# nz0001na/MorphGANformer

Measured on AMD Instinct MI355X. Metric: latent-projection iters/sec @1024^2, k=17 latents, higher is better.
Workload: dtype f32; 1 GPU; configs[1]: single 1024x1024 face per GPU, Wing+LPIPS(squeeze)+MSE literal-mode projection step, noise_mode=random, seeded synthetic weights/targets/landmarks; k=17, z_dim=32, targets_per_gpu=1, parallelism=pair-sharded x1, graph_replay=True, loss_generator_overlap=True, steps_per_forward=32

## Files before the change

include/mgf.h:

```cpp
#ifndef MGF_H_
#define MGF_H_

#include <stdint.h>

#ifdef __cplusplus
extern "C" {
#endif

typedef void* mgf_stream_t;

enum { MGF_OK = 0, MGF_EINVAL = -1, MGF_EUNSUPPORTED = -2, MGF_ELAUNCH = -3, MGF_ETOOBIG = -4 };
enum { MGF_F32 = 0, MGF_F64 = 1, MGF_F16 = 2 };
enum { MGF_FILTER_SEPARABLE = 2 };
enum { MGF_FILTER_LARGE = 4 };
enum { MGF_ACT_LINEAR = 1, MGF_ACT_RELU = 2, MGF_ACT_LRELU = 3, MGF_ACT_TANH = 4, MGF_ACT_SIGMOID = 5,
       MGF_ACT_ELU = 6, MGF_ACT_SELU = 7, MGF_ACT_SOFTPLUS = 8, MGF_ACT_SWISH = 9,
       MGF_ACT_RELU_POST = 10 };

const char* mgf_last_error(void);
int mgf_version(void);
int mgf_device_ok(void);

int mgf_bias_act(void* y, const void* x, const void* b, const void* xref, const void* yref, const void* dy,
                 int dtype, int64_t numel, int64_t step_b, int64_t size_b,
// ... 66 lines not shown
                                  const float* rgb_w, const float* rgb_bias, int32_t n, int32_t cin, int32_t h, int32_t w, int32_t cout,
                                  int32_t out_scale_stride, int32_t rgb_channels, mgf_stream_t stream);
int mgf_conv3x3_winograd2_f32(float* y, const float* x, const float* u, const float* in_scale, const float* out_scale, int32_t n,
                              int32_t cin, int32_t h, int32_t w, int32_t cout, int32_t out_scale_stride, const mgf_epilogue* ep,
                              mgf_stream_t stream);
int mgf_conv3x3_winograd3_f32(float* y, const float* x, const float* u, const float* in_scale, const float* out_scale, int32_t n,
                              int32_t cin, int32_t h, int32_t w, int32_t cout, int32_t out_scale_stride, const mgf_epilogue* ep,
                              mgf_stream_t stream);
int mgf_conv3x3_winograd3_slice_f32(float* y, const float* x, const float* u, const float* in_scale, const float* out_scale, int32_t n,
                                    int32_t cin, int32_t h, int32_t w, int32_t cout, int32_t out_scale_stride, int64_t y_batch,
                                    int32_t y_choff, const mgf_epilogue* ep, mgf_stream_t stream);
int mgf_conv1x1_f32(float* y, const float* x, const float* w, const float* in_scale, int32_t n, int32_t cin, int32_t hw, int32_t cout,
                    int32_t cout_pad, int64_t y_batch, int32_t y_choff, const mgf_epilogue* ep, mgf_stream_t stream);
int mgf_conv1x1_force_shape(int32_t channel_blocks);

int mgf_conv3x3s2_few_inputs_f32(float* y, const float* x, const float* w, const float* bias, int32_t n, int32_t cin, int32_t in_h,
                                 int32_t in_w, int32_t cout, int32_t relu, mgf_stream_t stream);
int mgf_tconv3x3s2_few_outputs_f32(float* y, const float* x, const float* wp, int32_t n, int32_t cin, int32_t h, int32_t w, int32_t cout,
                                   int32_t cout_pad, int32_t pitch, int64_t y_plane, int64_t y_batch, mgf_stream_t stream);
int mgf_conv3x3_winograd3_up2res_f32(float* y, const float* x, const float* u, const float* in_scale, const float* out_scale,
                                     const float* residual_low, int32_t n, int32_t cin, int32_t h, int32_t w, int32_t cout,
                                     int32_t out_scale_stride, const mgf_epilogue* ep, mgf_stream_t stream);
int mgf_winograd3_force_shape(int32_t shape);
int mgf_conv3x3_winograd3_rgb_f32(float* rgb_out, const float* x, const float* u, const float* in_scale, const float* out_scale,
                                  const float* rgb_w, const float* rgb_bias, int32_t n, int32_t cin, int32_t h, int32_t w, int32_t cout,
                                  int32_t out_scale_stride, int32_t rgb_channels, mgf_stream_t stream);
int mgf_conv3x3_winograd_f32(float* y, const float* x, const float* u, const float* in_scale, const float* out_scale, int32_t n,
                             int32_t cin, int32_t h, int32_t w, int32_t cout, int32_t out_scale_stride, const mgf_epilogue* ep,
                             mgf_stream_t stream);

int mgf_tconv3x3s2_border_f32(float* t, const float* x, const float* wp, const float* in_scale, const float* out_scale, int32_t n,
                              int32_t cin, int32_t h, int32_t w, int32_t cout, int32_t cout_pad, int64_t t_pitch, int64_t t_plane,
                              int64_t t_batch, int64_t out_scale_stride, mgf_stream_t stream);

int mgf_tconv3x3s2_winograd_f32(float* t, const float* x, const float* u, const float* in_scale, const float* out_scale, int32_t n,
                                int32_t cin, int32_t h, int32_t w, int32_t cout, int32_t pitch, int64_t t_plane, int64_t t_batch,
                                int64_t out_scale_stride, mgf_stream_t stream);
int mgf_tconv_winograd_weights_f32(float* u, const float* w, int32_t cout, int32_t cin, double gain, mgf_stream_t stream);

int mgf_pack_conv_weights(float* wp, float* wsq, const float* w, int32_t cout, int32_t cin, int32_t kh, int32_t kw,
                          int32_t cout_pad, float gain, int32_t flip, mgf_stream_t stream);

typedef struct mgf_style_job {
    const float* aff_w;
    const float* aff_b;
    const float* wsq;
    float* s;
    float* d;
    int32_t cin, cout;
    int32_t w_offset;
    float aff_gain, style_gain;
} mgf_style_job;
int mgf_demod_f32(float* d, const float* s, const float* wsq, int32_t n, int32_t cin, int32_t cout, mgf_stream_t stream);
int mgf_demod_bwd_f32(float* ds, const float* dd, const float* d, const float* s, const float* wsq, int32_t n, int32_t cin, int32_t cout,
                      mgf_stream_t stream);
int mgf_style_demod(const mgf_style_job* job, const float* ws, int64_t ws_stride_n, int32_t n, int32_t wdim, mgf_stream_t stream);
int mgf_style_demod_multi(const mgf_style_job* jobs_dev, int32_t njobs, const float* ws, int64_t ws_stride_n,
                          int32_t n, int32_t wdim, int32_t max_cin, mgf_stream_t stream);

int mgf_duplex_attention(float* y, const float* x, const float* wqc, const float* spos, const float* vwb,
                         int32_t n, int32_t c, int32_t f, int32_t t,
                         const mgf_epilogue* ep, int32_t ep_w, float* probs, int32_t* argmax, mgf_stream_t stream);

int mgf_att_map_upsample_f32(float* out, const float* probs, int32_t n, int32_t side, int32_t t, int32_t out_res, int32_t layer,
                             int32_t n_layers, mgf_stream_t stream);

// ... 226 lines not shown
```

morphganformer_amd/_lib.py:

```python
from __future__ import annotations

import ctypes as C
import os

import torch

HERE = os.path.dirname(os.path.abspath(__file__))
LIB_PATH = os.environ.get("MGF_LIB_PATH") or os.path.join(HERE, "libmgf_hip.so")

MGF_F32, MGF_F64, MGF_F16 = 0, 1, 2
ACT_IDS = {"linear": 1, "relu": 2, "lrelu": 3, "tanh": 4, "sigmoid": 5, "elu": 6, "selu": 7, "softplus": 8, "swish": 9,
           "relu_post": 10}
MAX_TAPS = 9

i32, i64, f32, f64, vp = C.c_int32, C.c_int64, C.c_float, C.c_double, C.c_void_p


class Epilogue(C.Structure):
    _fields_ = [("bias", vp), ("noise", vp), ("noise_strength", vp), ("noise_n", i32), ("act", i32), ("alpha", f32),
                ("gain", f32), ("residual", vp)]


class ConvDesc(C.Structure):
    _fields_ = [("n", i32), ("cin", i32), ("in_h", i32), ("in_w", i32), ("cout", i32), ("cout_pad", i32),
# ... 11 lines not shown
class StyleJob(C.Structure):
    _fields_ = [("aff_w", vp), ("aff_b", vp), ("wsq", vp), ("s", vp), ("d", vp), ("cin", i32), ("cout", i32),
                ("w_offset", i32), ("aff_gain", f32), ("style_gain", f32)]


class AttnJob(C.Structure):
    _fields_ = [("wmv", vp), ("bmv", vp), ("vwb", vp), ("c", i32), ("w_offset", i32)]


class StyleBwdJob(C.Structure):
    _fields_ = [("aff_w", vp), ("wsq", vp), ("s", vp), ("d", vp), ("ds_part", vp), ("dc_part", vp), ("cin", i32), ("cout", i32),
                ("s_chunks", i32), ("d_chunks", i32), ("aff_gain", f32), ("style_gain", f32)]


class AttnGradJob(C.Structure):
    _fields_ = [("dg", vp), ("probs", vp), ("dc", vp), ("cpre", vp), ("part", vp), ("dvwb", vp), ("dc_part", vp), ("c", i32), ("f", i32),
                ("slices", i32), ("nchunk", i32), ("blk_grad", i32), ("blk_dot", i32), ("blk_red", i32), ("pad_", i32)]


class AttnBwdJob(C.Structure):
    _fields_ = [("wmv", vp), ("dvwb", vp), ("c", i32), ("pad_", i32)]


_SIGS = {
    "mgf_last_error": (C.c_char_p, []),
    "mgf_version": (C.c_int, []),
    "mgf_device_ok": (C.c_int, []),
    "mgf_bias_act": (C.c_int, [vp, vp, vp, vp, vp, vp, C.c_int, i64, i64, i64, C.c_int, C.c_int, f32, f32, f32, vp]),
    "mgf_upfirdn2d": (C.c_int, [vp, vp, vp, C.c_int, i32, i32, i32, i32, i64, i64, i64, i64, i32, i32, i64, i64, i64, i64,
                                i32, i32, i32, i32, i32, i32, i32, i32, i32, i32, i32, f32, C.POINTER(Epilogue), vp]),
    "mgf_conv_taps_f32": (C.c_int, [vp, vp, vp, vp, vp, C.POINTER(ConvDesc), C.POINTER(Epilogue), vp]),
    "mgf_conv_taps_bf16x3_f32": (C.c_int, [vp, vp, vp, vp, vp, C.POINTER(ConvDesc), C.POINTER(Epilogue), vp]),
    "mgf_tconv3x3s2_border_f32": (C.c_int, [vp, vp, vp, vp, vp, i32, i32, i32, i32, i32, i32, i64, i64, i64, i64, vp]),
    "mgf_tconv3x3s2_winograd_f32": (C.c_int, [vp, vp, vp, vp, vp, i32, i32, i32, i32, i32, i32, i64, i64, i64, vp]),
    "mgf_tconv_winograd_weights_f32": (C.c_int, [vp, vp, i32, i32, C.c_double, vp]),
    "mgf_winograd_weights_f32": (C.c_int, [vp, vp, i32, i32, f32, vp]),
    "mgf_conv3x3_winograd_f32": (C.c_int, [vp, vp, vp, vp, vp, i32, i32, i32, i32, i32, i32, C.POINTER(Epilogue), vp]),
    "mgf_winograd2_weights_f32": (C.c_int, [vp, vp, i32, i32, f32, vp]),
    "mgf_conv3x3_winograd2_f32": (C.c_int, [vp, vp, vp, vp, vp, i32, i32, i32, i32, i32, i32, C.POINTER(Epilogue), vp]),
    "mgf_conv3x3_winograd2_rgb_f32": (C.c_int, [vp, vp, vp, vp, vp, vp, vp, i32, i32, i32, i32, i32, i32, i32, vp]),
    "mgf_conv3x3_winograd3_f32": (C.c_int, [vp, vp, vp, vp, vp, i32, i32, i32, i32, i32, i32, C.POINTER(Epilogue), vp]),
    "mgf_conv1x1_f32": (C.c_int, [vp, vp, vp, vp, i32, i32, i32, i32, i32, i64, i32, C.POINTER(Epilogue), vp]),
    "mgf_conv3x3s2_few_inputs_f32": (C.c_int, [vp, vp, vp, vp, i32, i32, i32, i32, i32, i32, vp]),
    "mgf_tconv3x3s2_few_outputs_f32": (C.c_int, [vp, vp, vp, i32, i32, i32, i32, i32, i32, i32, i64, i64, vp]),
    "mgf_conv1x1_force_shape": (C.c_int, [i32]),
    "mgf_conv3x3_winograd3_slice_f32": (C.c_int, [vp, vp, vp, vp, vp, i32, i32, i32, i32, i32, i32, i64, i32, C.POINTER(Epilogue), vp]),
    "mgf_conv3x3_winograd3_up2res_f32": (C.c_int, [vp, vp, vp, vp, vp, vp, i32, i32, i32, i32, i32, i32, C.POINTER(Epilogue), vp]),
    "mgf_winograd3_force_shape": (C.c_int, [i32]),
    "mgf_conv3x3_winograd3_rgb_f32": (C.c_int, [vp, vp, vp, vp, vp, vp, vp, i32, i32, i32, i32, i32, i32, i32, vp]),
    "mgf_conv3x3_winograd2_slice_f32": (C.c_int, [vp, vp, vp, vp, vp, i32, i32, i32, i32, i32, i32, i64, i32, C.POINTER(Epilogue), vp]),
    "mgf_pack_conv_weights": (C.c_int, [vp, vp, vp, i32, i32, i32, i32, i32, f32, i32, vp]),
    "mgf_conv_profile_begin": (C.c_int, []),
    "mgf_conv_profile_end": (C.c_int, [C.POINTER(ConvProfRec), i32]),
    "mgf_demod_f32": (C.c_int, [vp, vp, vp, i32, i32, i32, vp]),
    "mgf_demod_bwd_f32": (C.c_int, [vp, vp, vp, vp, vp, i32, i32, i32, vp]),
    "mgf_style_demod": (C.c_int, [C.POINTER(StyleJob), vp, i64, i32, i32, vp]),
    "mgf_style_demod_multi": (C.c_int, [vp, i32, vp, i64, i32, i32, i32, vp]),
    "mgf_duplex_attention": (C.c_int, [vp, vp, vp, vp, vp, i32, i32, i32, i32, C.POINTER(Epilogue), i32, vp, vp, vp]),
    "mgf_att_map_upsample_f32": (C.c_int, [vp, vp, i32, i32, i32, i32, i32, i32, vp]),
    "mgf_attn_values": (C.c_int, [C.POINTER(AttnJob), vp, i64, i64, i32, i32, i32, vp]),
    "mgf_attn_values_multi": (C.c_int, [vp, i32, vp, i64, i64, i32, i32, i32, vp]),
    "mgf_randn_f32": (C.c_int, [vp, i64, C.c_uint64, vp, vp]),
    "mgf_rgb_weights_f32": (C.c_int, [vp, vp, vp, i32, i32, i32, vp]),
    "mgf_torgb_compose_weights_f32": (C.c_int, [vp, vp, vp, vp, vp, vp, i32, i32, i32, i32, vp]),
    "mgf_conv3x3_few_outputs_f32": (C.c_int, [vp, vp, vp, vp, i32, i32, i32, i32, i32, vp]),
    "mgf_mapping_param_floats": (i64, [i32, i32, i32]),
# ... 151 lines not shown
```

morphganformer_amd/build.py:

```python
from __future__ import annotations

import glob
import hashlib
import os
import subprocess
import sys

HERE = os.path.dirname(os.path.abspath(__file__))
ROOT = os.path.dirname(HERE)
CSRC = os.path.join(HERE, "csrc")
OBJ = os.path.join(CSRC, "_obj")
LIB = os.path.join(HERE, "libmgf_hip.so")
SOURCES = ["capi.cpp", "bias_act.hip", "upfirdn2d.hip", "conv_taps.hip", "latent_prep.hip", "attention.hip", "losses.hip", "lpips_stem.hip",
           "embed.hip", "backward.hip", "wino.hip", "wino3.hip", "pointwise.hip", "narrow_conv.hip", "warp.hip", "lbp.hip", "mdf.hip",
           "wino_tconv.hip", "depthwise.hip", "noise_opt.hip", "morph_pair.hip"]
HEADERS = [os.path.join(CSRC, "mgf_common.h"), os.path.join(ROOT, "include", "mgf.h")]
HIPCC = os.environ.get("HIPCC", "/opt/rocm/bin/hipcc")
FLAGS = ["--offload-arch=gfx950", "-O3", "-fPIC", "-std=c++17", "-ffp-contract=on", "-Wno-unused-result", "-x", "hip"]
LINK_FLAGS = ["--offload-arch=gfx950", "-shared", "-fPIC"]

_compiler_id = None


def compiler_id() -> str:
    global _compiler_id
    if _compiler_id is None:
        _compiler_id = subprocess.run([HIPCC, "--version"], stdout=subprocess.PIPE, stderr=subprocess.STDOUT, check=True).stdout.decode()
    return _compiler_id


def object_key(src_path: str, flags) -> str:
    h = hashlib.sha256()
    h.update(compiler_id().encode())
    h.update("\0".join(flags).encode())
    for p in [src_path] + HEADERS:
        with open(p, "rb") as f:
            h.update(b"\0" + os.path.basename(p).encode() + b"\0" + f.read())
    return h.hexdigest()[:16]


def _compile_all(obj_dir, flags_for, verbose, force, prune=True):
    os.makedirs(obj_dir, exist_ok=True)
    objs, todo = [], []
    for src in SOURCES:
        sp = os.path.join(CSRC, src)
        flags = flags_for(src)
        op = os.path.join(obj_dir, f"{src}.{object_key(sp, flags)}.o")
        objs.append(op)
# ... 95 lines not shown
```

morphganformer_amd/conv.py:

```python
from __future__ import annotations

import ctypes as C
import os
from dataclasses import dataclass

import torch

from . import _lib


def round_up(v: int, m: int) -> int:
    return (v + m - 1) // m * m


def profile_begin():
    _lib.check(_lib.lib().mgf_conv_profile_begin(), "conv_profile_begin")


def profile_end(max_recs=4096):
    recs = (_lib.ConvProfRec * max_recs)()
    n = _lib.lib().mgf_conv_profile_end(recs, max_recs)
    if n < 0:
        _lib.check(n, "conv_profile_end")
    return [(recs[i].kernel.decode(), recs[i].flops, recs[i].seconds, recs[i].ksplit, recs[i].bytes) for i in range(min(n, max_recs))]
# ... 407 lines not shown
        _lib.check(rc, "tconv3x3s2_few_outputs")
        return out[:, :, :, :ow]
    if wt is not None and tconv_winograd_ok(n, cin, h, w, pc.cout, out, bf):
        assert tuple(wt.shape) == (25, cin // 4, pc.cout, 4)
        os_stride = 0 if out_scale is None else out_scale.stride(0) if out_scale.ndim == 2 else 0
        rc = _lib.lib().mgf_tconv3x3s2_winograd_f32(out.data_ptr(), x.data_ptr(), wt.data_ptr(), _lib.ptr(in_scale), _lib.ptr(out_scale), n, cin, h,
                                                    w, pc.cout, pitch, oh * pitch, pc.cout * oh * pitch, os_stride, _lib.stream_ptr())
        _lib.check(rc, "tconv3x3s2_winograd")
        rc = _lib.lib().mgf_tconv3x3s2_border_f32(out.data_ptr(), x.data_ptr(), pc.wp.data_ptr(), _lib.ptr(in_scale), _lib.ptr(out_scale),
                                                  n, cin, h, w, pc.cout, pc.cout_pad, pitch, oh * pitch, pc.cout * oh * pitch, os_stride,
                                                  _lib.stream_ptr())
        _lib.check(rc, "tconv3x3s2_border")
        return out[:, :, :, :ow]
    split = SPLIT_TCONV_BORDER and min(h, w) >= (TCONV_SPLIT_MIN if n >= 4 else max(TCONV_SPLIT_MIN, 128))
    use_bf = bf is not None and split and w % 32 == 0 and cin % 16 == 0
    os_stride = 0 if out_scale is None else out_scale.stride(0) if out_scale.ndim == 2 else 0
    d = _desc(n, cin, h, w, pc.cout, pc.cout_pad, h if split else h + 1, w if split else w + 1, 1, 2, TCONV_TAPS, TCONV_GROUPS,
              [0, 0, 1, 1], [0, 1, 0, 1], oh, ow, pitch, oh * pitch, pc.cout * oh * pitch, 0, os_stride)
    if use_bf:
        rc = _lib.lib().mgf_conv_taps_bf16x3_f32(out.data_ptr(), x.data_ptr(), bf.data_ptr(), _lib.ptr(in_scale), _lib.ptr(out_scale),
                                                 C.byref(d), None, _lib.stream_ptr())
    else:
        rc = _lib.lib().mgf_conv_taps_f32(out.data_ptr(), x.data_ptr(), pc.wp.data_ptr(), _lib.ptr(in_scale), _lib.ptr(out_scale),
                                          C.byref(d), None, _lib.stream_ptr())
    _lib.check(rc, "conv_taps(tconv)")
    if split:
        rc = _lib.lib().mgf_tconv3x3s2_border_f32(out.data_ptr(), x.data_ptr(), pc.wp.data_ptr(), _lib.ptr(in_scale), _lib.ptr(out_scale),
                                                  n, cin, h, w, pc.cout, pc.cout_pad, pitch, oh * pitch, pc.cout * oh * pitch, os_stride,
                                                  _lib.stream_ptr())
        _lib.check(rc, "tconv3x3s2_border")
    return out[:, :, :, :ow]


def upfirdn_into(y, x, f2d, up=1, pad=(0, 0, 0, 0), gain=1.0, flip=False, epilogue=None, separable=False, down=1):
    _lib.require_gpu(x, y, f2d)
    n, c, h, w = x.shape
    fh, fw = f2d.shape
    px0, px1, py0, py1 = pad
    oh = (h * up + py0 + py1 - fh + down) // down
    ow = (w * up + px0 + px1 - fw + down) // down
    assert tuple(y.shape) == (n, c, oh, ow), (tuple(y.shape), (n, c, oh, ow))
    sx, sy = x.stride(), y.stride()
    rc = _lib.lib().mgf_upfirdn2d(y.data_ptr(), x.data_ptr(), f2d.data_ptr(), _lib.MGF_F32, n, c, h, w, sx[0], sx[1], sx[2],
                                  sx[3], oh, ow, sy[0], sy[1], sy[2], sy[3], fh, fw, up, up, down, down, px0, px1, py0, py1,
                                  int(flip) | (2 if separable else 0) | 4,
                                  float(gain), C.byref(epilogue) if epilogue is not None else None,
                                  _lib.stream_ptr())
    _lib.check(rc, "upfirdn2d")
    return y
```

morphganformer_amd/engine.py:

```python
from __future__ import annotations

import ctypes as C
import math
import os
from dataclasses import dataclass, field

import numpy as np
import torch

from . import _lib
from . import conv as cv
from .synth_weights import GeneratorConfig

SQRT2 = math.sqrt(2.0)
SQRT_HALF = math.sqrt(0.5)
USE_WINOGRAD = os.environ.get("MGF_WINOGRAD", "1") != "0"
WINOGRAD_MAX_RES = int(os.environ.get("MGF_WINOGRAD_MAX_RES", "1024"))
TCONV_WINO_MAX_RES = int(os.environ.get("MGF_TCONV_WINO_MAX_RES", "256"))
BF_DIRECT_MAX_RES = int(os.environ.get("MGF_BF_DIRECT_MAX_RES", "128"))


def pack_mapping_params(sd, cfg: GeneratorConfig) -> np.ndarray:
    D, T = cfg.w_dim, cfg.k - 1
    lr = cfg.mapping_lrmul
# ... 54 lines not shown
    w_gained: torch.Tensor = None
    wino_u: torch.Tensor = None
    wino_t: torch.Tensor = None
    pcb: torch.Tensor = None
    s_off: int = 0
    d_off: int = 0


@dataclass
class AttnPlan:
    c: int
    f: int
    wqc: torch.Tensor
    spos: torch.Tensor
    wmv: torch.Tensor
    bmv: torch.Tensor
    v_off: int = 0


class SynthesisPlan:

    def __init__(self, sd, cfg: GeneratorConfig, device="cuda", arith="f32"):
        _lib.lib()
        self.cfg = cfg
        self.arith = arith
        self.device = torch.device(device)
        dev = self.device
        f64 = lambda k: np.asarray(sd[k], dtype=np.float64)
        t32 = lambda a: torch.as_tensor(np.ascontiguousarray(a, dtype=np.float32), device=dev)
        D, T = cfg.w_dim, cfg.k - 1
        self.mapping_blob = t32(pack_mapping_params(sd, cfg))
        self.const = t32(f64("synthesis.b4.const"))
        self.fir = t32(f64(f"synthesis.b{cfg.block_resolutions[-1]}.resample_kernel"))
        self.fir_is_1331 = bool(np.allclose(f64(f"synthesis.b{cfg.block_resolutions[-1]}.resample_kernel"),
                                            np.outer([1, 3, 3, 1], [1, 3, 3, 1]) / 64.0, rtol=0, atol=1e-7))
        self.layers: list[ConvLayerPlan] = []
        self.skips = {}
        s_off = d_off = v_off = 0
        for (res, name, cin, cout, up, slot, att, has_nb) in cfg.layer_table():
            p = f"synthesis.b{res}.{name}"
            w = f64(p + ".weight")
            kind = "torgb" if name == "torgb" else ("tconv" if up == 2 else "conv3")
            lp = ConvLayerPlan(name=p, res=res, cin=cin, cout=cout, up=up, slot=slot, kind=kind)
            if kind == "torgb":
                lp.pc = cv.pack_weights(t32(w), gain=1.0, flip=False)
                lp.w_raw = t32(w.reshape(cout, cin))
                lp.style_gain = 1.0 / math.sqrt(cin)
                lp.demod = False
            else:
                wg = 1.0 / math.sqrt(cin * 9)
                lp.pc = cv.pack_weights(t32(w), gain=wg, flip=False, want_wsq=True)
                if kind == "conv3" and USE_WINOGRAD and cv.winograd_ok(cin, cout, res, res) and res <= WINOGRAD_MAX_RES:
                    lp.wino_u = cv.winograd_pack(t32(w), wg, res)
                if (kind == "tconv" and arith != "bf16x3" and cv.TCONV_WINO and res <= TCONV_WINO_MAX_RES and cin % 4 == 0
                        and cout % 32 == 0):
                    lp.wino_t = cv.tconv_winograd_weights(t32(w), wg)
                if arith == "bf16x3" and cin % 16 == 0 and res // up >= 32:
                    lp.pcb = cv.pack_weights_bf16x3(lp.pc)
            lp.aff_w = t32(f64(p + ".affine.weight"))
            lp.aff_b = t32(f64(p + ".affine.bias"))
            if (p + ".biasAct.bias") in sd:
                lp.bias = t32(f64(p + ".biasAct.bias"))
            if (p + ".noise_strength") in sd:
                lp.noise_strength = t32(f64(p + ".noise_strength").reshape(1))
                lp.noise_const = t32(f64(p + ".noise_const"))
            lp.act_gain = SQRT2 * (SQRT_HALF if (name == "conv1" and res > 4) else 1.0)
# ... 426 lines not shown

    def _draw_noise(self, n):
        sizes = [(lp.name, lp.res) for lp in self.plan.layers if lp.noise_strength is not None]
        total = sum(r * r for _, r in sizes)
        if self.noise_rand is None or self.noise_rand.numel() != n * total:
            self.noise_rand = torch.empty(n * total, dtype=torch.float32, device=self.device)
        if not torch.cuda.is_current_stream_capturing():
            gen = torch.cuda.default_generators[self.device.index if self.device.index is not None else torch.cuda.current_device()]
            seed, off = int(gen.initial_seed()), int(gen.get_offset())
            if (seed, off) != self._noise_epoch:
                self.noise_seed = (seed ^ (off * 0x9E3779B97F4A7C15)) & 0xFFFFFFFFFFFFFFFF
                self.noise_state.zero_()
            gen.set_offset(off + 4)
            self._noise_epoch = (seed, off + 4)
        _lib.check(_lib.lib().mgf_randn_f32(self.noise_rand.data_ptr(), self.noise_rand.numel(), self.noise_seed, self.noise_state.data_ptr(),
                                            _lib.stream_ptr()), "randn")
        out, off = {}, 0
        for name, r in sizes:
            out[name] = self.noise_rand[off * n:(off + r * r) * n].view(n, r * r)
            off += r * r
        return out

    def _bf_direct(self, lp, n, residual_low):
        return (lp.pcb is not None and lp.kind == "conv3" and residual_low is None and 32 <= lp.res <= BF_DIRECT_MAX_RES
                and n * (lp.res // 8) * (lp.res // 32) * (lp.cout // 32) >= 512)

    def _layer(self, lp, x, B, key, noise_mode, noises, residual, residual_low=None):
        n = x.shape[0]
        noise, noise_n = self._noise_for(lp, noise_mode, noises)
        ep = _lib.make_epilogue(bias=lp.bias, noise=noise, noise_strength=lp.noise_strength if noise is not None else None,
                                noise_n=noise_n, act="lrelu", alpha=0.2, gain=lp.act_gain, residual=residual)
        has_att = lp.attn is not None
        s, d = self._s(lp), self._d(lp)
        if lp.kind == "tconv":
            t = cv.tconv3x3s2_forward(x, lp.pc, in_scale=s, out_scale=d, out=B["t"], bf=lp.pcb, wt=lp.wino_t)
            y = cv.upfirdn_into(B[key], t, self.plan.fir, up=1, pad=(1, 1, 1, 1), gain=4.0, epilogue=None if has_att else ep,
                                separable=True)
        elif self._bf_direct(lp, n, residual_low):
            y = cv.conv_forward(x, lp.pc, pad=(1, 1), in_scale=s, out_scale=d, epilogue=None if has_att else ep, out=B[key], bf=lp.pcb)
        elif lp.wino_u is not None and cv.winograd_fills_chip(n, lp.cout, lp.res, lp.res):
            y = cv.winograd_forward(x, lp.wino_u, in_scale=s, out_scale=d, epilogue=None if has_att else ep, out=B[key],
                                    residual_low=residual_low)
        else:
            y = cv.conv_forward(x, lp.pc, pad=(1, 1), in_scale=s, out_scale=d, epilogue=None if has_att else ep, out=B[key])
        if self.taps is not None:
            self.taps[lp.name + ":conv"] = y
        if has_att:
            a = lp.attn
            out = B[key + "a"]
            probs = argmax = None
            if self.att_maps is not None:
                probs = torch.empty([n, a.f, self.cfg.k - 1], dtype=torch.float32, device=self.device)
                argmax = torch.empty([n, a.f], dtype=torch.int32, device=self.device)
                self.att_maps[lp.name] = (probs, argmax)
            rc = _lib.lib().mgf_duplex_attention(out.data_ptr(), y.data_ptr(), a.wqc.data_ptr(), a.spos.data_ptr(),
                                                 self._v(lp).data_ptr(), n, a.c, a.f, self.cfg.k - 1, C.byref(ep), lp.res,
                                                 _lib.ptr(probs), _lib.ptr(argmax), _lib.stream_ptr())
            _lib.check(rc, "duplex_attention")
            y = out
        return y

    def forward_workspace(self, z=None, c=None, ws=None, truncation_psi=1, truncation_cutoff=None, return_img=True, return_att=False,
                          return_ws=False, subnet=None, noise_mode="random", noises=None, fused_modconv=None, att_format="tensor", lean=False):
        lean = bool(lean) and self.taps is None and not return_att
        nb = (z if ws is None else ws)
        if nb is not None and (nb.shape[0], lean) != (self.n, self.lean):
            self._alloc(nb.shape[0], lean)
# ... 37 lines not shown
```

Measured before the change: 781.0 iters/s.

## Fuse stride-2 transposed conv with separable FIR blur and epilogue in one kernel

Adds a HIP kernel that computes the 3x3 stride-2 transposed convolution with MFMA and then applies the separable upsampling FIR blur, noise, bias, leaky-ReLU and gain straight from registers and LDS. Work is split into row steps with a carry buffer between them. This removes the intermediate tensor write and read and a separate upfirdn launch for tconv layers that have small cin, no attention and no winograd path. It adds a large, complex kernel with its own eligibility checks and falls back to the old two-kernel path otherwise.

```diff
diff --git a/include/mgf.h b/include/mgf.h
--- a/include/mgf.h
+++ b/include/mgf.h
@@ -122,6 +122,10 @@
 int mgf_tconv3x3s2_border_f32(float* t, const float* x, const float* wp, const float* in_scale, const float* out_scale, int32_t n,
                               int32_t cin, int32_t h, int32_t w, int32_t cout, int32_t cout_pad, int64_t t_pitch, int64_t t_plane,
                               int64_t t_batch, int64_t out_scale_stride, mgf_stream_t stream);
+
+int mgf_tconv3x3s2_blur_f32(float* y, const float* x, const float* wp, const float* in_scale, const float* out_scale, const float* f1d,
+                            float gain, int32_t n, int32_t cin, int32_t h, int32_t w, int32_t cout, int32_t cout_pad, int64_t y_pitch,
+                            int64_t y_plane, int64_t y_batch, int64_t out_scale_stride, const mgf_epilogue* ep, mgf_stream_t stream);
 
 int mgf_tconv3x3s2_winograd_f32(float* t, const float* x, const float* u, const float* in_scale, const float* out_scale, int32_t n,
                                 int32_t cin, int32_t h, int32_t w, int32_t cout, int32_t pitch, int64_t t_plane, int64_t t_batch,
diff --git a/morphganformer_amd/_lib.py b/morphganformer_amd/_lib.py
--- a/morphganformer_amd/_lib.py
+++ b/morphganformer_amd/_lib.py
@@ -67,6 +67,7 @@
     "mgf_conv_taps_f32": (C.c_int, [vp, vp, vp, vp, vp, C.POINTER(ConvDesc), C.POINTER(Epilogue), vp]),
     "mgf_conv_taps_bf16x3_f32": (C.c_int, [vp, vp, vp, vp, vp, C.POINTER(ConvDesc), C.POINTER(Epilogue), vp]),
     "mgf_tconv3x3s2_border_f32": (C.c_int, [vp, vp, vp, vp, vp, i32, i32, i32, i32, i32, i32, i64, i64, i64, i64, vp]),
+    "mgf_tconv3x3s2_blur_f32": (C.c_int, [vp, vp, vp, vp, vp, vp, C.c_float, i32, i32, i32, i32, i32, i32, i64, i64, i64, i64, C.POINTER(Epilogue), vp]),
     "mgf_tconv3x3s2_winograd_f32": (C.c_int, [vp, vp, vp, vp, vp, i32, i32, i32, i32, i32, i32, i64, i64, i64, vp]),
     "mgf_tconv_winograd_weights_f32": (C.c_int, [vp, vp, i32, i32, C.c_double, vp]),
     "mgf_winograd_weights_f32": (C.c_int, [vp, vp, i32, i32, f32, vp]),
diff --git a/morphganformer_amd/build.py b/morphganformer_amd/build.py
--- a/morphganformer_amd/build.py
+++ b/morphganformer_amd/build.py
@@ -13,7 +13,7 @@
 LIB = os.path.join(HERE, "libmgf_hip.so")
 SOURCES = ["capi.cpp", "bias_act.hip", "upfirdn2d.hip", "conv_taps.hip", "latent_prep.hip", "attention.hip", "losses.hip", "lpips_stem.hip",
            "embed.hip", "backward.hip", "wino.hip", "wino3.hip", "pointwise.hip", "narrow_conv.hip", "warp.hip", "lbp.hip", "mdf.hip",
-           "wino_tconv.hip", "depthwise.hip", "noise_opt.hip", "morph_pair.hip"]
+           "wino_tconv.hip", "depthwise.hip", "noise_opt.hip", "morph_pair.hip", "tconv_blur.hip"]
 HEADERS = [os.path.join(CSRC, "mgf_common.h"), os.path.join(ROOT, "include", "mgf.h")]
 HIPCC = os.environ.get("HIPCC", "/opt/rocm/bin/hipcc")
 FLAGS = ["--offload-arch=gfx950", "-O3", "-fPIC", "-std=c++17", "-ffp-contract=on", "-Wno-unused-result", "-x", "hip"]
diff --git a/morphganformer_amd/conv.py b/morphganformer_amd/conv.py
--- a/morphganformer_amd/conv.py
+++ b/morphganformer_amd/conv.py
@@ -463,6 +463,60 @@
     return out[:, :, :, :ow]
 
 
+TCONV_BLUR = os.environ.get("MGF_TCONV_BLUR", "1") != "0"
+TCONV_BLUR_MIN_WGS = 512
+TCONV_BLUR_MAX_CIN = 64
+
+
+def tconv_blur_wgs(n, h, w, cout) -> int:
+    return min(512, n * -(-w // 30) * (cout // 32) * ((2 * h + 2 + 15) // 16))
+
+
+def fir_factor(f2d: torch.Tensor):
+    f = f2d.detach().double().cpu()
+    if tuple(f.shape) != (4, 4) or not float(f[0, 0]) > 0:
+        return None
+    a = f[:, 0] / f[0, 0].sqrt()
+    if not torch.allclose(torch.outer(a, a), f, rtol=1e-6, atol=0):
+        return None
+    return a.float().to(f2d.device)
+
+
+def tconv_blur_ok(n, cin, h, w, cout, out, f1d, epilogue=None, bf=None) -> bool:
+    if not TCONV_BLUR or bf is not None or f1d is None or cin % 8 != 0 or cout % 32 != 0 or cin > TCONV_BLUR_MAX_CIN:
+        return False
+    if epilogue is not None and (epilogue.residual or (epilogue.act == _lib.ACT_IDS["lrelu"] and not 0.0 <= epilogue.alpha <= 1.0)
+                                 or epilogue.act not in (0, _lib.ACT_IDS["linear"], _lib.ACT_IDS["lrelu"])):
+        return False
+    st = out.stride()
+    if out.dim() != 4 or st[3] != 1 or st[1] >= 1 << 28 or cin * h * w >= 1 << 28 or st[0] % 2 or st[1] % 2 or st[2] % 2 or out.data_ptr() % 8:
+        return False
+    return tconv_blur_wgs(n, h, w, cout) >= TCONV_BLUR_MIN_WGS
+
+
+def tconv3x3s2_blur_forward(x, pc: PackedConv, f1d, gain, in_scale=None, out_scale=None, epilogue=None, out=None, t=None, f2d=None,
+                            bf=None, wt=None):
+    _lib.require_gpu(x, pc.wp, in_scale, out_scale, out, f1d)
+    assert pc.kh == 3 and pc.kw == 3 and x.dtype == torch.float32 and x.is_contiguous()
+    n, cin, h, w = x.shape
+    if out is None:
+        out = torch.empty([n, pc.cout, 2 * h, 2 * w], dtype=torch.float32, device=x.device)
+    assert tuple(out.shape) == (n, pc.cout, 2 * h, 2 * w) and out.dtype == torch.float32
+    if tconv_blur_ok(n, cin, h, w, pc.cout, out, f1d, epilogue, bf):
+        sy = out.stride()
+        os_stride = 0 if out_scale is None else out_scale.stride(0) if out_scale.ndim == 2 else 0
+        rc = _lib.lib().mgf_tconv3x3s2_blur_f32(out.data_ptr(), x.data_ptr(), pc.wp.data_ptr(), _lib.ptr(in_scale), _lib.ptr(out_scale),
+                                                f1d.data_ptr(), float(gain), n, cin, h, w, pc.cout, pc.cout_pad, sy[2], sy[1], sy[0],
+                                                os_stride, C.byref(epilogue) if epilogue is not None else None, _lib.stream_ptr())
+        if rc != -2:
+            _lib.check(rc, "tconv3x3s2_blur")
+            return out
+    if f2d is None:
+        f2d = torch.outer(f1d, f1d)
+    tt = tconv3x3s2_forward(x, pc, in_scale=in_scale, out_scale=out_scale, out=t, bf=bf, wt=wt)
+    return upfirdn_into(out, tt, f2d, up=1, pad=(1, 1, 1, 1), gain=gain, epilogue=epilogue, separable=True)
+
+
 def upfirdn_into(y, x, f2d, up=1, pad=(0, 0, 0, 0), gain=1.0, flip=False, epilogue=None, separable=False, down=1):
     _lib.require_gpu(x, y, f2d)
     n, c, h, w = x.shape
diff --git a/morphganformer_amd/csrc/tconv_blur.hip b/morphganformer_amd/csrc/tconv_blur.hip
--- /dev/null
+++ b/morphganformer_amd/csrc/tconv_blur.hip
@@ -0,0 +1,385 @@
+#include "mgf_common.h"
+
+namespace {
+
+typedef float f32x16 __attribute__((ext_vector_type(16)));
+
+constexpr int CK = 8;
+#ifndef MGF_TB_ABL
+#define MGF_TB_ABL 0
+#endif
+constexpr int OWN = (MGF_TB_ABL & 2) ? 32 : 30;
+constexpr int FW = 33, FH = 9, CHS = FH * FW;
+constexpr int XS = 10, WS = 3;
+constexpr int XS_REGION = XS * 256, BUF = XS_REGION + WS * 1024;
+constexpr int SLICE = 8 * 16 * 64;
+constexpr int CARRY = 32 * 3 * 64;
+constexpr int LDS_FLOATS = 2 * BUF + CARRY + 64;
+static_assert(SLICE <= 2 * BUF, "the slice lives in the staging buffers");
+static_assert(LDS_FLOATS * 4 <= 80 * 1024, "two workgroups per CU");
+
+struct Ones8 { float v[8]; };
+__device__ const Ones8 g_ones8 = {{1.f, 1.f, 1.f, 1.f, 1.f, 1.f, 1.f, 1.f}};
+
+struct TBParams {
+    float* y;
+    const float* x;
+    const float* wp;
+    const float* in_scale;
+    const float* out_scale;
+    const float* f1d;
+    float gain;
+    int n, cin, h, w, cout_pad;
+    int y_pitch, y_plane;
+    int64_t y_batch, os_stride;
+    mgf_epilogue ep;
+    int strips, cot, steps;
+    int total, per;
+};
+
+struct Unit { int n, co0, j0, s; };
+
+__device__ __forceinline__ float dpp_from_left(float v) {
+    return __builtin_bit_cast(float, __builtin_amdgcn_mov_dpp(__builtin_bit_cast(int, v), 0x138, 0xf, 0xf, true));
+}
+__device__ __forceinline__ float dpp_from_right(float v) {
+    return __builtin_bit_cast(float, __builtin_amdgcn_mov_dpp(__builtin_bit_cast(int, v), 0x130, 0xf, 0xf, true));
+}
+
+__global__ __launch_bounds__(256, 2) void tconv_blur_kernel(TBParams p) {
+    extern __shared__ float lds[];
+    float* const carry = lds + 2 * BUF;
+    float* const prm = carry + CARRY;
+    const int tid = threadIdx.x, tid_ = tid, lane = tid & 63, wave = __builtin_amdgcn_readfirstlane(tid >> 6);
+    const int l31 = lane & 31, half = lane >> 5;
+    const int plane = p.h * p.w;
+
+    const int vb = (int)(blockIdx.x & 7) * (int)(gridDim.x >> 3) + (int)(blockIdx.x >> 3);
+    const int g_begin = vb * p.per;
+    int g_end = g_begin + p.per;
+    if (g_end > p.total) g_end = p.total;
+    if (g_begin >= g_end) return;
+    const int u0 = g_begin - ((g_begin % p.steps) != 0 ? 1 : 0);
+
+    auto decode = [&](int u, Unit& c) {
+        const int item = u / p.steps;
+        c.s = u - item * p.steps;
+        const int ct = item % p.cot;
+        const int r = item / p.cot;
+        const int strip = r % p.strips;
+        c.n = r / p.strips;
+        c.co0 = ct * 32;
+        c.j0 = strip * OWN;
+        c.n = __builtin_amdgcn_readfirstlane(c.n); c.co0 = __builtin_amdgcn_readfirstlane(c.co0);
+        c.j0 = __builtin_amdgcn_readfirstlane(c.j0); c.s = __builtin_amdgcn_readfirstlane(c.s);
+    };
+
+    float fx[3], fy[4];
+    {
+        const float f0 = p.f1d[0];
+#pragma unroll
+        for (int t = 0; t < 3; ++t) fx[t] = p.f1d[3 - t] / f0;
+#pragma unroll
+        for (int t = 0; t < 4; ++t) fy[t] = p.f1d[3 - t] * f0 * p.gain;
+    }
+
+    f32x16 acc[4][2];
+    auto zero_acc = [&]() {
+#pragma unroll
+        for (int q = 0; q < 4; ++q)
+#pragma unroll
+            for (int g = 0; g < 2; ++g)
+#pragma unroll
+                for (int r = 0; r < 16; ++r) acc[q][g][r] = 0.f;
+    };
+    zero_acc();
+
+    unsigned xoff[XS];
+    int woff[WS], wch[WS];
+    __amdgpu_buffer_rsrc_t rx_l = __builtin_amdgcn_make_buffer_rsrc((void*)p.x, 0, 0, 0x00020000);
+    const __amdgpu_buffer_rsrc_t rw_l = __builtin_amdgcn_make_buffer_rsrc((void*)p.wp, 0, (int)(4u * (unsigned)(9 * p.cin * p.cout_pad)), 0x00020000);
+    __amdgpu_buffer_rsrc_t rs_l = __builtin_amdgcn_make_buffer_rsrc((void*)g_ones8.v, 0, 32, 0x00020000);
+    const int sc_step = p.in_scale ? 4 : 0;
+    auto setup_slots = [&](const Unit& c) {
+        rx_l = __builtin_amdgcn_make_buffer_rsrc((void*)(p.x + (int64_t)c.n * p.cin * plane), 0, (int)(4u * (unsigned)(p.cin * plane)), 0x00020000);
+        if (p.in_scale) rs_l = __builtin_amdgcn_make_buffer_rsrc((void*)(p.in_scale + (int64_t)c.n * p.cin), 0, 4 * p.cin, 0x00020000);
+        int tid = tid_;
+        asm volatile("" : "+v"(tid));
+#pragma unroll
+        for (int j = 0; j < WS; ++j) {
+            int i = tid + 256 * j;
+            if (i >= 576) i = 575;
+            const int c4 = i & 7, rest = i >> 3;
+            wch[j] = rest & 7;
+            woff[j] = ((rest >> 3) * p.cin + wch[j]) * p.cout_pad + c.co0 + c4 * 4;
+        }
+        const int iy0 = c.s * 8 - 1, ix0 = c.j0 - 2;
+#pragma unroll
+        for (int j = 0; j < XS; ++j) {
+            const int i = tid + 256 * j;
+            const int ch = i / CHS, rem = i - ch * CHS;
+            const int r = rem / FW, q = rem - r * FW;
+            const int iy = iy0 + r, ix = ix0 + q;
+            xoff[j] = (i < CK * CHS && iy >= 0 && iy < p.h && ix >= 0 && ix < p.w) ? 4u * (unsigned)(ch * plane + iy * p.w + ix) : 0xFFFFFFF0u;
+        }
+    };
+    float xr[XS];
+    float4 wr[WS];
+    float wsc[WS];
+    auto load_chunk = [&](int c0) {
+        const int xso = (int)(4u * (unsigned)(c0 * plane)), wso = (int)(4u * (unsigned)(c0 * p.cout_pad)), sso = c0 * sc_step;
+#pragma unroll
+        for (int j = 0; j < XS; ++j) xr[j] = __builtin_bit_cast(float, __builtin_amdgcn_raw_buffer_load_b32(rx_l, xoff[j], xso, 0));
+#pragma unroll
+        for (int j = 0; j < WS; ++j) {
+            wr[j] = __builtin_bit_cast(float4, __builtin_amdgcn_raw_buffer_load_b128(rw_l, 4u * (unsigned)woff[j], wso, 0));
+            wsc[j] = __builtin_bit_cast(float, __builtin_amdgcn_raw_buffer_load_b32(rs_l, 4u * (unsigned)wch[j], sso, 0));
+        }
+    };
+    auto store_chunk = [&](float* buf) {
+#pragma unroll
+        for (int j = 0; j < XS; ++j) buf[tid + 256 * j] = xr[j];
+        float* Wd = buf + XS_REGION;
+#pragma unroll
+        for (int j = 0; j < WS; ++j) {
+            float4 v = wr[j];
+            v.x *= wsc[j]; v.y *= wsc[j]; v.z *= wsc[j]; v.w *= wsc[j];
+            *reinterpret_cast<float4*>(Wd + (tid + 256 * j) * 4) = v;
+        }
+    };
+    const int pb0 = (wave * 2) * FW + l31, pb1 = pb0 + FW;
+    auto mfma_chunk = [&](const float* buf) {
+        auto toff = [](int t) { return ((t / 3) == 2 ? 0 : FW) + ((t % 3) == 2 ? 0 : 1); };
+        const float* Xs = buf + half * CHS;
+        const float* Ws = buf + XS_REGION + half * 32 + l31;
+        float fa[2][CK / 2], fb[2][CK / 2][2];
+        auto fetch = [&](int t, int set) {
+#pragma unroll
+            for (int kk = 0; kk < CK / 2; ++kk) {
+                fa[set][kk] = Ws[(t * CK + 2 * kk) * 32];
+                fb[set][kk][0] = Xs[2 * kk * CHS + pb0 + toff(t)];
+                fb[set][kk][1] = Xs[2 * kk * CHS + pb1 + toff(t)];
+            }
+        };
+        fetch(0, 0);
+#pragma unroll
+        for (int t = 0; t < 9; ++t) {
+            if (t + 1 < 9) {
+                fetch(t + 1, (t + 1) & 1);
+#pragma unroll
+                for (int i = 0; i < (CK / 2) * 3; ++i) {
+                    __builtin_amdgcn_sched_group_barrier(0x008, 1, 0);
+                    __builtin_amdgcn_sched_group_barrier(0x100, 1, 0);
+                }
+            }
+            const int q = ((t / 3) == 1 ? 2 : 0) + ((t % 3) == 1 ? 1 : 0);
+#pragma unroll
+            for (int kk = 0; kk < CK / 2; ++kk)
+#pragma unroll
+                for (int g = 0; g < 2; ++g)
+                    acc[q][g] = __builtin_amdgcn_mfma_f32_32x32x2f32(fa[t & 1][kk], fb[t & 1][kk][g], acc[q][g], 0, 0, 0);
+        }
+    };
+
+    const bool has_noise = p.ep.noise != nullptr;
+    const float ep_ns = has_noise ? (p.ep.noise_strength ? *p.ep.noise_strength : 1.0f) : 0.f;
+    const float alpha = p.ep.act == MGF_ACT_LRELU ? p.ep.alpha : 1.0f, egain = p.ep.gain;
+    const int out_h = 2 * p.h, out_w = 2 * p.w;
+
+    auto blur = [&](const Unit& c, bool emit) {
+        float2 nz[4];
+        float* const S = lds;
+        const int ycol = 2 * (c.j0 - 1) + 2 * l31;
+        const bool col_ok = (MGF_TB_ABL & 2) ? (ycol >= 0 && ycol < out_w) : (l31 >= 1 && l31 < 31 && ycol < out_w);
+        const int R0 = 16 * c.s - 2 + 4 * wave;
+        float* const yb = p.y + (int64_t)c.n * p.y_batch + (int64_t)c.co0 * p.y_plane;
+        uint32_t yo[4];
+#pragma unroll
+        for (int j = 0; j < 4; ++j) {
+            const bool ok = emit && col_ok && R0 + j >= 0 && R0 + j < out_h && !(MGF_TB_ABL & 4);
+            yo[j] = ok ? 4u * (uint32_t)(half * p.y_plane + (R0 + j) * p.y_pitch + ycol) : 0xFFFFFFF0u;
+        }
+        const int laneS = (half * 16 + 4 * wave - 3) * 64 + 2 * l31, laneC = 2 * BUF + half * 192 + 2 * l31;
+        const int laneLow = wave == 0 ? laneC : laneS;
+        float* const Sw = S + ((4 * half) * 16 + 4 * wave) * 64 + 2 * l31;
+#pragma unroll
+        for (int k = 0; k < 4; ++k) {
+#pragma unroll
+            for (int g = 0; g < 2; ++g)
+#pragma unroll
+                for (int a = 0; a < 2; ++a)
+#pragma unroll
+                    for (int rr = 0; rr < 4; ++rr) {
+                        const float E = acc[2 * a][g][4 * k + rr], O = acc[2 * a + 1][g][4 * k + rr];
+                        const float Ol = dpp_from_left(O), Er = dpp_from_right(E), Or = dpp_from_right(O);
+                        float he = __builtin_fmaf(fx[2], O, Er);
+                        he = __builtin_fmaf(fx[1], E, he);
+                        he = __builtin_fmaf(fx[0], Ol, he);
+                        float ho = __builtin_fmaf(fx[2], Er, Or);
+                        ho = __builtin_fmaf(fx[1], O, ho);
+                        ho = __builtin_fmaf(fx[0], E, ho);
+                        asm("" : "+v"(he), "+v"(ho));
+                        *reinterpret_cast<float2*>(Sw + (rr * 16 + 2 * g + a) * 64) = make_float2(he, ho);
+                    }
+            if (k == 0) {
+#pragma unroll
+                for (int j = 0; j < 4; ++j) nz[j] = make_float2(0.f, 0.f);
+                if (has_noise) {
+                    const int ycol = 2 * (c.j0 - 1) + 2 * l31;
+                    const int R0 = 16 * c.s - 2 + 4 * wave;
+                    const float* nb = p.ep.noise + (int64_t)(p.ep.noise_n > 1 ? c.n : 0) * out_h * out_w;
+#pragma unroll
+                    for (int j = 0; j < 4; ++j)
+                        if (l31 >= 1 && l31 < 31 && ycol < out_w && R0 + j >= 0 && R0 + j < out_h) {
+                            const float* q = nb + (int64_t)(R0 + j) * out_w + ycol;
+                            nz[j] = make_float2(q[0] * ep_ns, q[1] * ep_ns);
+                        }
+                }
+            }
+            __syncthreads();
+            float2 Bn[7];
+            float2 pn;
+            auto fetch_rows = [&](int it) {
+                const int lowoff = wave == 0 ? ((8 * k + 2 * it) * 3) * 64 : (2 * it * 16) * 64;
+#pragma unroll
+                for (int i = 0; i < 7; ++i)
+                    Bn[i] = *reinterpret_cast<const float2*>(i < 3 ? lds + laneLow + lowoff + i * 64 : S + laneS + (2 * it * 16 + i) * 64);
+                pn = make_float2(prm[8 * k + 2 * it + half], prm[32 + 8 * k + 2 * it + half]);
+            };
+            fetch_rows(0);
+#pragma unroll
+            for (int it = 0; it < 4; ++it) {
+                float2 B[7];
+#pragma unroll
+                for (int i = 0; i < 7; ++i) B[i] = Bn[i];
+                const float dsc = pn.x, bia = pn.y;
+                if (it + 1 < 4) fetch_rows(it + 1);
+                const int ch = 8 * k + 2 * it;
+                const __amdgpu_buffer_rsrc_t ry = __builtin_amdgcn_make_buffer_rsrc((void*)(yb + (int64_t)ch * p.y_plane), 0, 8 * p.y_plane, 0x00020000);
+#pragma unroll
+                for (int j = 0; j < 4; ++j) {
+                    float o0 = B[j].x * fy[0], o1 = B[j].y * fy[0];
+                    o0 = __builtin_fmaf(B[j + 1].x, fy[1], o0); o1 = __builtin_fmaf(B[j + 1].y, fy[1], o1);
+                    o0 = __builtin_fmaf(B[j + 2].x, fy[2], o0); o1 = __builtin_fmaf(B[j + 2].y, fy[2], o1);
+                    o0 = __builtin_fmaf(B[j + 3].x, fy[3], o0); o1 = __builtin_fmaf(B[j + 3].y, fy[3], o1);
+                    float v0 = __builtin_fmaf(o0, dsc, nz[j].x), v1 = __builtin_fmaf(o1, dsc, nz[j].y);
+                    v0 += bia; v1 += bia;
+                    v0 = __builtin_fmaxf(v0, v0 * alpha);
+                    v1 = __builtin_fmaxf(v1, v1 * alpha);
+                    v0 *= egain; v1 *= egain;
+                    asm("" : "+v"(v0), "+v"(v1));
+                    typedef unsigned u32x2 __attribute__((ext_vector_type(2)));
+                    u32x2 pk = {__builtin_bit_cast(unsigned, v0), __builtin_bit_cast(unsigned, v1)};
+                    __builtin_amdgcn_raw_buffer_store_b64(pk, ry, yo[j], 0, 0);
+                }
+            }
+            __syncthreads();
+            if (wave == 3) {
+#pragma unroll
+                for (int e = 0; e < 12; ++e) {
+                    const int row = 2 * e + half, cl = row / 3, i = row - 3 * cl;
+                    const float2 v = *reinterpret_cast<const float2*>(S + (cl * 16 + 13 + i) * 64 + 2 * l31);
+                    *reinterpret_cast<float2*>(carry + ((8 * k + cl) * 3 + i) * 64 + 2 * l31) = v;
+                }
+            }
+            if (k == 3) __syncthreads();
+        }
+    };
+
+    Unit cur;
+    decode(u0, cur);
+    int b = 0;
+    setup_slots(cur);
+    load_chunk(0);
+    store_chunk(lds);
+    __syncthreads();
+    const int nch = p.cin / CK;
+    for (int u = u0;; ++u) {
+        if (cur.s == 0 || u == u0) {
+            for (int i = tid; i < CARRY; i += 256) carry[i] = 0.f;
+        }
+        if (tid < 32) {
+            prm[tid] = p.out_scale ? p.out_scale[(int64_t)cur.n * p.os_stride + cur.co0 + tid] : 1.0f;
+            prm[32 + tid] = p.ep.bias ? p.ep.bias[cur.co0 + tid] : 0.f;
+        }
+        for (int c = 0; c + 1 < nch; ++c) {
+            load_chunk((c + 1) * CK);
+            mfma_chunk(lds + b * BUF);
+            store_chunk(lds + (b ^ 1) * BUF);
+            __syncthreads();
+            b ^= 1;
+        }
+        const bool have_next = u + 1 < g_end;
+        Unit nx = cur;
+        if (have_next) {
+            decode(u + 1, nx);
+            setup_slots(nx);
+            load_chunk(0);
+        }
+        mfma_chunk(lds + b * BUF);
+        __syncthreads();
+        if (MGF_TB_ABL & 1) {
+            if (p.gain == 12345.f) p.y[tid] = acc[0][0][0] + acc[1][1][5] + acc[2][0][10] + acc[3][1][15];
+        } else {
+            blur(cur, u >= g_begin);
+        }
+        zero_acc();
+        if (!have_next) break;
+        store_chunk(lds);
+        b = 0;
+        __syncthreads();
+        cur = nx;
+    }
+}
+
+}
+
+extern "C" int mgf_tconv3x3s2_blur_f32(float* y, const float* x, const float* wp, const float* in_scale, const float* out_scale,
+                                       const float* f1d, float gain, int32_t n, int32_t cin, int32_t h, int32_t w, int32_t cout,
+                                       int32_t cout_pad, int64_t y_pitch, int64_t y_plane, int64_t y_batch, int64_t out_scale_stride,
+                                       const mgf_epilogue* ep, mgf_stream_t stream) {
+    MGF_REQUIRE(y && x && wp && f1d, MGF_EINVAL, "tconv3x3s2_blur: null pointer");
+    MGF_REQUIRE(n >= 1 && cin >= 1 && h >= 1 && w >= 1 && cout >= 1 && cout_pad >= cout, MGF_EINVAL, "tconv3x3s2_blur: bad shape");
+    MGF_REQUIRE(cin % CK == 0 && cout % 32 == 0 && cout_pad % 32 == 0, MGF_EUNSUPPORTED,
+                "tconv3x3s2_blur: needs cin %% 8 == 0 and cout %% 32 == 0 (got %d, %d)", cin, cout);
+    MGF_REQUIRE(y_pitch >= 2 * (int64_t)w && y_plane >= 2 * (int64_t)h * y_pitch && y_batch >= (int64_t)cout * y_plane, MGF_EINVAL,
+                "tconv3x3s2_blur: output strides too small");
+    MGF_REQUIRE(y_pitch % 2 == 0 && y_plane % 2 == 0 && y_batch % 2 == 0 && ((uintptr_t)y % 8) == 0, MGF_EUNSUPPORTED,
+                "tconv3x3s2_blur: output needs even pitch / plane / batch strides and 8-byte alignment (column pairs are stored as float2)");
+    MGF_REQUIRE((int64_t)cin * h * w < (1LL << 28) && (int64_t)9 * cin * cout_pad < (1LL << 28) && y_plane < (1LL << 28),
+                MGF_ETOOBIG, "tconv3x3s2_blur: tensor too large");
+    if (ep) {
+        MGF_REQUIRE(!ep->residual, MGF_EUNSUPPORTED, "tconv3x3s2_blur: no residual port");
+        MGF_REQUIRE(ep->act == 0 || ep->act == MGF_ACT_LINEAR || (ep->act == MGF_ACT_LRELU && ep->alpha >= 0.f && ep->alpha <= 1.f), MGF_EUNSUPPORTED,
+                    "tconv3x3s2_blur: epilogue activation %d (slope %g) unsupported", ep->act, (double)ep->alpha);
+    }
+    TBParams p;
+    p.y = y; p.x = x; p.wp = wp; p.in_scale = in_scale; p.out_scale = out_scale; p.f1d = f1d; p.gain = gain;
+    p.n = n; p.cin = cin; p.h = h; p.w = w; p.cout_pad = cout_pad;
+    p.y_pitch = (int)y_pitch; p.y_plane = (int)y_plane; p.y_batch = y_batch; p.os_stride = out_scale_stride;
+    if (ep) { p.ep = *ep; if (p.ep.act == 0) p.ep.act = MGF_ACT_LINEAR; } else { p.ep = mgf_epilogue{}; p.ep.act = MGF_ACT_LINEAR; p.ep.gain = 1.f; }
+    p.strips = (int)mgf_cdiv(w, OWN);
+    p.cot = cout / 32;
+    p.steps = (2 * h + 2 + 15) / 16;
+    const int64_t total = (int64_t)n * p.strips * p.cot * p.steps;
+    MGF_REQUIRE(total <= INT32_MAX - 4096, MGF_ETOOBIG, "tconv3x3s2_blur: too many work units");
+    p.total = (int)total;
+    int64_t grid = (int64_t)MGF_NUM_CU * 2;
+    if (total < grid) grid = mgf_cdiv(total, 8) * 8;
+    p.per = (int)mgf_cdiv(total, grid);
+    static bool attr_set = false;
+    if (!attr_set) {
+        hipError_t e = hipFuncSetAttribute((const void*)tconv_blur_kernel, hipFuncAttributeMaxDynamicSharedMemorySize, LDS_FLOATS * 4);
+        if (e != hipSuccess) { mgf_set_error("tconv3x3s2_blur: cannot raise dynamic LDS: %s", hipGetErrorString(e)); return MGF_ELAUNCH; }
+        attr_set = true;
+    }
+    hipStream_t st = (hipStream_t)stream;
+    const double flops = 2.0 * 9 * cin * (double)cout * h * w * n;
+    const double bytes = 4.0 * ((double)n * cin * h * w + 9.0 * cin * cout + ((ep && ep->noise) ? (double)(ep->noise_n > 1 ? n : 1) * 4.0 * h * w : 0.0) +
+                                (double)n * cout * 4.0 * h * w);
+    mgf_prof_external_begin(st, "tconv_blur_kernel", flops, bytes);
+    hipLaunchKernelGGL(tconv_blur_kernel, dim3((unsigned)grid), dim3(256), LDS_FLOATS * 4, st, p);
+    mgf_prof_external_end(st);
+    MGF_CHECK_LAUNCH("tconv3x3s2_blur");
+    return MGF_OK;
+}
diff --git a/morphganformer_amd/engine.py b/morphganformer_amd/engine.py
--- a/morphganformer_amd/engine.py
+++ b/morphganformer_amd/engine.py
@@ -110,6 +110,7 @@
         self.mapping_blob = t32(pack_mapping_params(sd, cfg))
         self.const = t32(f64("synthesis.b4.const"))
         self.fir = t32(f64(f"synthesis.b{cfg.block_resolutions[-1]}.resample_kernel"))
+        self.fir1 = cv.fir_factor(self.fir)
         self.fir_is_1331 = bool(np.allclose(f64(f"synthesis.b{cfg.block_resolutions[-1]}.resample_kernel"),
                                             np.outer([1, 3, 3, 1], [1, 3, 3, 1]) / 64.0, rtol=0, atol=1e-7))
         self.layers: list[ConvLayerPlan] = []
@@ -602,7 +603,12 @@
                                 noise_n=noise_n, act="lrelu", alpha=0.2, gain=lp.act_gain, residual=residual)
         has_att = lp.attn is not None
         s, d = self._s(lp), self._d(lp)
-        if lp.kind == "tconv":
+        if (lp.kind == "tconv" and not has_att and self.taps is None and lp.pcb is None
+                and cv.tconv_blur_ok(n, x.shape[1], x.shape[2], x.shape[3], lp.cout, B[key], self.plan.fir1, ep)
+                and not (lp.wino_t is not None and cv.tconv_winograd_ok(n, x.shape[1], x.shape[2], x.shape[3], lp.cout, B["t"]))):
+            y = cv.tconv3x3s2_blur_forward(x, lp.pc, self.plan.fir1, 4.0, in_scale=s, out_scale=d, epilogue=ep, out=B[key], t=B["t"],
+                                           f2d=self.plan.fir, wt=lp.wino_t)
+        elif lp.kind == "tconv":
             t = cv.tconv3x3s2_forward(x, lp.pc, in_scale=s, out_scale=d, out=B["t"], bf=lp.pcb, wt=lp.wino_t)
             y = cv.upfirdn_into(B[key], t, self.plan.fir, up=1, pad=(1, 1, 1, 1), gain=4.0, epilogue=None if has_att else ep,
                                 separable=True)
```

Measured after the change: 800.5 iters/s (median of 6 runs). +2.5%, better.
